# Meowuu7/equi-articulated-pose

Measured on AMD Instinct MI355X. Metric: point-clouds/sec (4096 pts, 60 anchors) fwd+bwd, higher is better.
Workload: dtype f32; 1 GPU; 8 x 4096-pt synthetic laptop clouds per GPU, 3-block inter backbone 1->64->128->512 (NN=64,K=24,A=60), forward+backward+Adam; clouds_per_gpu=8, points=4096, anchors=60

## Files before the change

### equi-articulated-pose_amd/vgtk/_hip.py

```python
import ctypes
import os
import weakref

import torch

_PKG_ROOT = os.path.abspath(os.path.join(os.path.dirname(__file__), '..'))
LIB_PATH = os.path.join(_PKG_ROOT, 'libeap_hip.so')

if not os.path.exists(LIB_PATH):
    raise ImportError(
        f'{LIB_PATH} not found: build the HIP extension first '
        '(python -c "import __graft_entry__ as g; g.build()" or make -C equi-articulated-pose_amd/csrc). '
        'This package has no CPU fallback.')

lib = ctypes.CDLL(LIB_PATH)
lib.eap_last_error.restype = ctypes.c_char_p
lib.eap_last_kernel.restype = ctypes.c_char_p
lib.eap_gemm_f32_reduce_workspace.restype = ctypes.c_int64
lib.eap_so3_inter_group_bwd_workspace.restype = ctypes.c_int64
lib.eap_inter_zpconv_fwd_workspace.restype = ctypes.c_int64
lib.eap_inter_zpconv_bwd_workspace.restype = ctypes.c_int64
lib.eap_inter_zpconv_bwd_hot_workspace.restype = ctypes.c_int64
lib.eap_bn_act_segments.restype = ctypes.c_int

# ... 761 lines not shown
        return hint[0].sum(1, dtype=torch.float64), hint[1].sum(1, dtype=torch.float64)
    ps, pq = _partials(x, b, c, n)
    call('eap_bn_stats_f32', x, b, c, _I64(n), _ptr(x), _ptr(ps), _ptr(pq))
    return ps.sum(1, dtype=torch.float64), pq.sum(1, dtype=torch.float64)


def bn_act_fwd(x, b, c, n, scale, shift, slope, residual=None):
    y = torch.empty_like(x)
    if residual is None:
        call('eap_bn_act_fwd_f32', x, b, c, _I64(n), _F32(slope), _ptr(x), _ptr(scale), _ptr(shift), _ptr(y))
    else:
        call('eap_bn_act_add_fwd_f32', x, b, c, _I64(n), _F32(slope), _ptr(x), _ptr(scale), _ptr(shift), _ptr(residual), _ptr(y))
    return y


def bn_act_bwd_reduce(gy, x, b, c, n, scale, shift, mean, invstd, slope):
    pg, pgx = _partials(x, b, c, n)
    call('eap_bn_act_bwd_reduce_f32', x, b, c, _I64(n), _F32(slope), _ptr(gy), _ptr(x), _ptr(scale), _ptr(shift),
         _ptr(mean), _ptr(invstd), _ptr(pg), _ptr(pgx))
    return pg.sum(1, dtype=torch.float64), pgx.sum(1, dtype=torch.float64)


_ROWMAX_HINT = [None]
USE_ROWMAX_HINT = True
ROWMAX_HINTS_TAKEN = 0


def leave_rowmax_hint(t, rowmax):
    _leave_hint(_ROWMAX_HINT, t, rowmax)


def take_rowmax_hint(t):
    global ROWMAX_HINTS_TAKEN
    rowmax = _take_hint(_ROWMAX_HINT, t)
    ROWMAX_HINTS_TAKEN += rowmax is not None
    return rowmax


def bn_act_bwd_apply(gy, x, b, c, n, scale, shift, mean, invstd, k2, k3, slope):
    gx = torch.empty_like(x)
    if x.dim() == 4 and x.shape[3] % 4 == 0 and x.shape[3] <= 64 and n == x.shape[2] * x.shape[3] and c % 128 == 0 and gx.data_ptr() % 16 == 0 \
            and gy.data_ptr() % 16 == 0 and x.data_ptr() % 16 == 0:
        rowmax = torch.empty(b, c, x.shape[3], dtype=torch.int32, device=x.device)
        call('eap_bn_act_bwd_apply_rowmax_f32', x, b, c, _I64(n), int(x.shape[3]), _F32(slope), _ptr(gy), _ptr(x), _ptr(scale), _ptr(shift),
             _ptr(mean), _ptr(invstd), _ptr(k2), _ptr(k3), _ptr(gx), _ptr(rowmax))
        leave_rowmax_hint(gx, rowmax)
        return gx
    call('eap_bn_act_bwd_apply_f32', x, b, c, _I64(n), _F32(slope), _ptr(gy), _ptr(x), _ptr(scale), _ptr(shift),
         _ptr(mean), _ptr(invstd), _ptr(k2), _ptr(k3), _ptr(gx))
    return gx



def bn_stats_masked(x, b, c, n, na, mask):
    ps, pq = _partials(x, b, c, n)
    call('eap_bn_stats_masked_f32', x, b, c, _I64(n), na, _ptr(x), _ptr(mask), _ptr(ps), _ptr(pq))
    return ps.view(c, b, -1).sum(2, dtype=torch.float64).t(), pq.view(c, b, -1).sum(2, dtype=torch.float64).t()


def bn_act_cloud_fwd(x, b, c, n, scale, shift, slope):
    y = torch.empty_like(x)
    call('eap_bn_act_cloud_fwd_f32', x, b, c, _I64(n), _F32(slope), _ptr(x), _ptr(scale), _ptr(shift), _ptr(y))
    return y


def bn_act_cloud_bwd_reduce(gy, x, b, c, n, scale, shift, mean, invstd, slope):
    pg, pgx = _partials(x, b, c, n)
    call('eap_bn_act_cloud_bwd_reduce_f32', x, b, c, _I64(n), _F32(slope), _ptr(gy), _ptr(x), _ptr(scale), _ptr(shift),
         _ptr(mean), _ptr(invstd), _ptr(pg), _ptr(pgx))
    return pg.view(c, b, -1).sum(2, dtype=torch.float64).t(), pgx.view(c, b, -1).sum(2, dtype=torch.float64).t()


def bn_act_cloud_bwd_apply(gy, x, b, c, n, na, scale, shift, mean, invstd, k2, k3, mask, slope):
    gx = torch.empty_like(x)
    call('eap_bn_act_cloud_bwd_apply_f32', x, b, c, _I64(n), na, _F32(slope), _ptr(gy), _ptr(x), _ptr(scale), _ptr(shift),
         _ptr(mean), _ptr(invstd), _ptr(k2), _ptr(k3), _ptr(mask), _ptr(gx))
    return gx


def so3_intra_conv(feats, W, intra_idx32):
    b, c, p, na = feats.shape
    o, nt = W.shape[0], intra_idx32.shape[1]
    out = torch.empty(b, o, p, na, dtype=torch.float32, device=feats.device)
    split = SPLIT_BF16_CONTRACTION and W.data_ptr() % 16 == 0 and lib.eap_so3_intra_conv_bf16x3_f32_supported(b, o, c, p, na, nt)
    tag = {'flops': 2.0 * b * o * c * nt * p * na, 'shape': ('intra_conv', b, o, c, p, na, nt)}
    if split and SPLIT_PLANES == 2 and feats.data_ptr() % 16 == 0:
        abs_w = absmax_rows(W, 1, o, c * nt, c * nt, 0)
        abs_f = absmax_colgroups(feats, b, c, p * na, p * na, c * p * na, na) if na % 4 == 0 else None
        if abs_w is not None and abs_f is not None:
            call('eap_so3_intra_conv_f16x2_f32', out, b, o, c, p, na, nt, _ptr(W), _ptr(feats), _ptr(intra_idx32), _ptr(out), _ptr(abs_w),
                 _ptr(abs_f), tag=tag)
            return out
    call('eap_so3_intra_conv_bf16x3_f32' if split else 'eap_so3_intra_conv_f32', out, b, o, c, p, na, nt, _ptr(W), _ptr(feats),
         _ptr(intra_idx32), _ptr(out), tag=tag)
    return out
```

### equi-articulated-pose_amd/vgtk/so3conv/functional.py

```python
import math
import os
import weakref

import numpy as np
import torch

import vgtk
import vgtk.functional as fr
import vgtk.pc as pctk
import vgtk.spconv as zpconv
import vgtk.cuda.grouping as cuda_nn

from .. import _hip

inter_so3conv_feat_grouping = zpconv.inter_zpconv_grouping_naive
batched_index_select = zpconv.batched_index_select
batched_index_select_other = zpconv.batched_index_select_other

MATERIALIZE_INTER_W = False

GAMMA_SIZE = 3
ROOT = vgtk.__path__[0]
Rs, R_idx, canonical_relative = fr.icosahedron_so3(GAMMA_SIZE)
_KP = np.load(os.path.join(ROOT, 'data', 'anchors', 'constants.npz'))
# ... 412 lines not shown

def _inverse_lists(idx, gx, n_sup, ident, nonident=None):
    if nonident is None:
        nonident = (gx[..., 3].contiguous().view(torch.int32) != ident).flatten(1).any(1).to(torch.int32)
    head = _ListHead(idx, n_sup, nonident)
    rcap, any_nonident = head.decide()
    head.wait()
    ent_p, ent_gx = _hip.inv_lists_fill(idx, gx, head.rows, head.off, rcap)
    return (head.rows[:, :rcap].contiguous(), head.off[:, :rcap].contiguous(), head.cnt[:, :rcap].contiguous(),
            ent_p, ent_gx, rcap, not any_nonident)


X_LAYOUT = 'transposed'


X_CHUNK_CLOUDS = 8
_KEEP_X_HINT = {}


def _keep_x_hint(W):
    hit = _KEEP_X_HINT.get(id(W))
    return bool(hit is not None and hit[0]() is W and hit[1])


def _set_keep_x_hint(W, keep):
    if len(_KEEP_X_HINT) > 1024:
        _KEEP_X_HINT.clear()
    _KEEP_X_HINT[id(W)] = (weakref.ref(W), bool(keep))


class FoldedEpilogue:

    def __init__(self, scale, shift, slope, residual=None):
        self.scale, self.shift, self.slope, self.residual = scale.contiguous(), shift.contiguous(), float(slope), residual
        self.applied = False
        self.inference = not torch.is_grad_enabled()


class TrainEpilogue:

    def __init__(self, norm):
        self.norm = norm
        self.applied = False
        self.inference = False
        self.residual = None

    def moments(self, s1, s2, pivot, count):
        from .blocks import affine_from_moments, batch_moments, update_running_stats
        norm = self.norm
        mean, var, total = batch_moments(s1, s2, pivot, count, norm.sync)
        if norm.running_mean is not None:
            update_running_stats(norm.running_mean, norm.running_var, mean, var, total, norm.momentum)
        gamma = norm.weight.detach().double()
        scale, shift, _ = affine_from_moments(mean, var, gamma, norm.bias.detach(), norm.eps)
        inv_gamma = torch.where(gamma == 0, torch.zeros_like(gamma), 1.0 / gamma).float()
        self.saved = (scale, norm.bias.detach().float().clone(), inv_gamma.contiguous(), total)
        return scale.contiguous(), shift.contiguous(), float(norm.negative_slope)


def _contract_into(W, x, y, layout, epilogue=None, b0=0, x_bound=None):
    b, c, ks, p, na = x.shape
    o = W.shape[0]
    if layout == 2:
        xt = x.view(b, p * na, c * ks).transpose(1, 2)
    if epilogue is not None and layout == 2:
        res = None if epilogue.residual is None else epilogue.residual[b0:b0 + b]
        if _hip.matmul_epilogue(W, xt, y, epilogue.scale, epilogue.shift, epilogue.slope, res, b_bound=x_bound):
            epilogue.applied = True
            return
        if b0 > 0 and epilogue.applied:
            raise RuntimeError('folded epilogue: the slabs of one contraction took different kernels')
    if layout == 2:
        _hip.matmul(W, xt, y, b_bound=x_bound)
    elif layout == 1:
        _hip.gemm(0, 0, o, p * na, c * ks, W, c * ks, 0, x, p * na, c * ks * p * na, y, p * na, o * p * na, b, b_blocked=True)
    else:
        _hip.matmul(W, x.view(b, c * ks, p * na), y)


def _grouped_bound(feats, idx):
    if not (_hip.SPLIT_BF16_CONTRACTION and _hip.SPLIT_PLANES == 2):
        return None
    return _hip.so3_grouped_bound(feats, idx)


BACKWARD_LOG = None
FORWARD_LOG = None


DENSE_MODE = os.environ.get('EAP_DENSE', 'auto')
DENSE_ROW_FACTOR = 5.0
DENSE_MAX_GROUPS = 16.0
DENSE_MAX_GROUPS_WIDE = 16.0
DENSE_FWD_NARROW = True
FUSE_CONV_NORM = True


def _dense_rows(rcap, n):
    return (rcap + 15) & ~15


def _dense_wanted(head, o, p, na, ks, nn, n):
    if DENSE_MODE == 'off' or head is None or head.memb is None:
        return 0, False
    rcap, _ = head.decide()
    rp = _dense_rows(rcap, n)
    if rp <= 0 or rp > n or not head.dense_possible() or not _hip.so3_dense_supported(p, na, ks, rp, o):
# ... 212 lines not shown
    moments = affine = None
    if train_ep is not None:
        ep, moments = train_ep, train_ep.moments
    elif folded is not None and folded.residual is None:
        ep, affine = folded, (folded.scale, folded.shift, folded.slope)
    else:
        return _dense_forward(feats, W, rows, geo, p), None
    g, ldg, operand = _dense_operand(feats, W, rows, geo)
    y = _hip.so3_dense_fwd_bnact(g, geo, p, feats.shape[1], ldg, moments, operand=operand, o=W.shape[0], affine=affine)
    ep.applied = True
    return y, (None if train_ep is None else train_ep.saved + (float(train_ep.norm.negative_slope), bool(train_ep.norm.sync)))


def _forward_lists(feats, W, args, layout, keep, folded, head, fill):
    idx, gx, rk, mult, sigma, nonident = args.idx, args.gx, args.rk, args.mult, args.sigma, args.nonident
    b, c, n, na = feats.shape
    p, ks, o = idx.shape[1], rk.shape[1], W.shape[0]
    if fill:
        head.fill(idx, gx, n)
    y = torch.empty(b, o, p, na, dtype=torch.float32, device=feats.device)
    coset = _coset_tables(mult, args.ident) if (mult is not None and nonident is not None and layout == 2) else None
    x_bound = _grouped_bound(feats, idx) if layout == 2 else None
    step = max(1, b if keep else X_CHUNK_CLOUDS)
    tp = (not keep and STORE_ORDER_COLUMNS and layout == 2 and _hip.so3_group_fwd_tp_takes(c, na, ks)
          and (mult is None or (coset is not None and _hip.so3_group_perm_lists2_takes(c, na, ks, n))))
    Wc = W.index_select(1, _hip.so3_group_fwd_tp_columns(c, ks, W.device)) if tp else W
    x = None
    for b0 in range(0, b, step):
        b1 = min(b, b0 + step)
        x = _hip.so3_inter_group_fwd(feats[b0:b1], idx[b0:b1], gx[b0:b1], rk, mult, sigma,
                                     None if nonident is None else nonident[b0:b1], blocked=layout, coset=coset, store_order=tp)
        _contract_into(Wc, x, y[b0:b1].view(b1 - b0, o, p * na), layout, folded, b0,
                       x_bound=None if x_bound is None else (x_bound[b0:b1], na, 1.0))
        x = x if keep else None
    return y, x


def _forward_map(feats, W, args, keep, folded):
    idx, gx, rk, amap = args.idx, args.gx, args.rk, args.amap
    b, na = feats.shape[0], feats.shape[3]
    p, o = idx.shape[1], W.shape[0]
    y = torch.empty(b, o, p, na, dtype=torch.float32, device=feats.device)
    step = max(1, b if keep else X_CHUNK_CLOUDS)
    x = None
    for b0 in range(0, b, step):
        b1 = min(b, b0 + step)
        x = _hip.so3_inter_group_fwd_map(feats[b0:b1], idx[b0:b1], gx[b0:b1], rk, amap[b0:b1], args.sigma)
        _contract_into(W, x, y[b0:b1].view(b1 - b0, o, p * na), 0, folded, b0)
        x = x if keep else None
    return y, x



def _weight_operand(W, c, ks, pad_c=None):
    o = W.shape[0]
    W2 = W.view(o, c, ks).permute(1, 0, 2).reshape(c, o * ks).contiguous()
    if pad_c is not None and pad_c != c:
        W2 = torch.cat([W2, torch.zeros(pad_c - c, o * ks, dtype=torch.float32, device=W.device)])
    return W2


def _rows_grad_from_z(z, W2, c, rp, na, ldz, anchor_major, z_bound=None, reorder=None):
    b, (pad_c, oks) = z.shape[0], W2.shape
    gFc = torch.empty(b, pad_c, ldz, dtype=torch.float32, device=z.device)
    _hip.matmul(W2, z.view(b, oks, ldz), gFc, b_bound=z_bound)
    if anchor_major:
        return gFc[:, :c, :rp * na].reshape(b, c, na, rp).transpose(2, 3)
    gFc = gFc.view(b, c, rp, na)
    return gFc if reorder is None else _hip.anchor_reorder(gFc, reorder)


def _weight_grad_rows(z, fc4, o, ks, ldz, anchor_major, reorder=None):
    b, c, rp, na = fc4.shape
    if reorder is not None:
        fc4 = _hip.anchor_reorder(fc4, reorder)
    fc = fc4.transpose(2, 3).contiguous() if anchor_major else fc4
    return _weight_grad_from_z(z, fc.view(b, c, rp * na), b, c, o, ks, rp * na, ldz)



def _backward_dense(gy, W, feats, head, geo, bn, yact, need_f, need_w):
    b, c, n, na = feats.shape
    o, ks, p, rp = W.shape[0], geo.ks, gy.shape[2], geo.rp
    if BACKWARD_LOG is not None:
        BACKWARD_LOG.append({'channels': (c, o), 'support_rows': n, 'referenced_rows_max': int(rp), 'regime': 'dense rows',
                             **({'norm': 'in the node'} if bn is not None else {})})
    ra = na * rp
    pad_c = 128 if (c == 64 and bn is not None) else c
    ldz = _hip.dense_pitch(ra) if (pad_c % 128 == 0 and (o * ks) % 16 == 0 and need_f) else ra
    gF = gW = g_bn_w = g_bn_b = z_bound = None
    if bn is not None:
        k1, beta, inv_gamma, count, slope, sync = bn
        from .blocks import all_reduce_sums
        sg, sgx, gmax, xmax = _hip.bn_act_bwd_reduce_fromy(gy, yact, beta, inv_gamma, slope)
        g_bn_w, g_bn_b = sgx.float(), sg.float()
        tg, tgx = all_reduce_sums(sg, sgx, sync=sync)
        k2 = (k1.double() * tg / count).float()
        k3 = (k1.double() * tgx / count).float()
        coef = torch.stack([k1, k2, k3, beta, inv_gamma]).contiguous()
        bound = (k1.abs()[None, :, None] * gmax + k2.abs()[None, :, None] + k3.abs()[None, :, None] * xmax).contiguous()
        z = _hip.so3_dense_bwd_bn(gy, yact, geo, ldz, coef, bound, slope)
        if ldz % 4 == 0 and rp % 4 == 0:
            live = torch.arange(rp, device=gy.device)[None, :] < head.n_rows[:, None]
            cntf = torch.where(live, head.cnt[:, :rp], torch.zeros_like(head.cnt[:, :rp])).clamp(min=0, max=p).to(torch.float32)
            cols = bound.amax(1)[:, :, None] * cntf[:, None, :]
            words = torch.zeros(b, ldz // 4, dtype=torch.float32, device=gy.device)
# ... 88 lines not shown
        gx_ = torch.empty_like(x.view(b, ck, pa))
        Wt = W.t().contiguous()
        _hip.matmul(Wt, gy.view(b, o, pa), gx_)
        gF = _hip.so3_inter_group_bwd(gx_.view(b, c, ks, p, na), idx, gx, rk, mult, args.sigma, n, args.ident)
    return gF, gW


def _backward_map(gy, W, feats, x, args, need_f, need_w):
    b, c, n, na = feats.shape
    idx, gx, rk, amap = args.idx, args.gx, args.rk, args.amap
    p, ks = idx.shape[1], rk.shape[1]
    o, ck, pa = W.shape[0], c * ks, p * na
    gF = gW = None
    if need_w:
        if x is None:
            x = _hip.so3_inter_group_fwd_map(feats, idx, gx, rk, amap, args.sigma)
        gW = torch.empty_like(W)
        _hip.matmul_reduce(gy.view(b, o, pa), x.view(b, ck, pa).transpose(1, 2), gW)
    if need_f:
        gx_ = torch.empty(b, ck, pa, dtype=torch.float32, device=gy.device)
        Wt = W.t().contiguous()
        _hip.matmul(Wt, gy.view(b, o, pa), gx_)
        gF = _hip.so3_inter_group_bwd_map(gx_.view(b, c, ks, p, na), idx, gx, rk, amap, args.sigma, n)
    return gF, gW


class _InterConv(torch.autograd.Function):

    DIFFERENTIABLE = 4

    @staticmethod
    def forward(ctx, feats, W_param, bn_weight, bn_bias, args):
        feats = feats.contiguous()
        W = W_param.contiguous()
        idx, rk, mult, nonident = args.idx, args.rk, args.mult, args.nonident
        can = X_LAYOUT != 'reference' and _hip.so3_inter_group_fwd_can_block(
            feats.shape[1], feats.shape[2], feats.shape[3], rk.shape[1], mult is not None, nonident is not None)
        layout = 0 if not can else (2 if X_LAYOUT == 'transposed' else 1)
        _, c, n, na = feats.shape
        p, ks, o = idx.shape[1], rk.shape[1], W.shape[0]
        needs_grad = (ctx.needs_input_grad[0] or ctx.needs_input_grad[1]) and args.grad_mode
        train_ep = args.epilogue if isinstance(args.epilogue, TrainEpilogue) else None
        folded = None if train_ep is not None else args.epilogue
        if folded is not None and (needs_grad or not folded.inference):
            raise RuntimeError('a folded epilogue is an inference-time fusion: build and use it under torch.no_grad()')
        if args.amap is not None:
            if FORWARD_LOG is not None:
                FORWARD_LOG.append({'channels': (c, o), 'dense': False, 'parts': None, 'regime': 'anchor map'})
            y, x = _forward_map(feats, W, args, needs_grad and ctx.needs_input_grad[1], folded)
            ctx.bn, ctx.conv_args, ctx.head, ctx.layout, ctx.plan = None, args, None, 0, None
            ctx.W_param = weakref.ref(W_param)
            ctx.save_for_backward(W, x, idx, args.gx, rk, None, nonident, feats, None)
            return y
        lists_ok = BACKWARD_MODE != 'dx' and _inv_lists_supported(idx, n, na, ks)
        keep = needs_grad and (not lists_ok or _keep_x_hint(W_param))
        plan = _DensePlan(args, n, o, lists_ok, needs_grad, keep, folded)
        head = plan.head if needs_grad else None
        if FORWARD_LOG is not None:
            FORWARD_LOG.append({'channels': (c, o), 'dense': bool(plan.forward), 'parts': None if plan.parts is None else plan.parts.n})
        if plan.forward:
            bn_only = args.grad_mode and not needs_grad and (ctx.needs_input_grad[2] or ctx.needs_input_grad[3])
            y, ctx.bn = _forward_dense(feats, W, plan, p, train_ep if (FUSE_CONV_NORM and not bn_only) else None, folded)
            x, layout = None, 0
        else:
            fill = head is not None and plan.probed and not keep and plan.rp == 0
            y, x = _forward_lists(feats, W, args, layout, keep, folded, head, fill)
            ctx.bn = None
        ctx.conv_args, ctx.head, ctx.layout = args, head, layout
        ctx.plan = plan if (plan.rp > 0 and needs_grad) else None
        ctx.W_param = weakref.ref(W_param)
        ctx.save_for_backward(W, x, idx, args.gx, rk, mult, nonident, feats, y if (ctx.bn is not None and needs_grad) else None)
        return y

    @staticmethod
    def backward(ctx, gy):
        W, x, idx, gx, rk, mult, nonident, feats, yact = ctx.saved_tensors
        args, head, plan = ctx.conv_args, ctx.head, ctx.plan
        gy = gy.contiguous()
        n = feats.shape[2]
        need_f, need_w = ctx.needs_input_grad[0], ctx.needs_input_grad[1]
        g_bn_w = g_bn_b = None
        if args.amap is not None:
            if BACKWARD_LOG is not None:
                BACKWARD_LOG.append({'channels': (feats.shape[1], W.shape[0]), 'support_rows': n, 'referenced_rows_max': 0, 'regime': 'anchor map'})
            gF, gW = _backward_map(gy, W, feats, x, args, need_f, need_w)
        elif plan is not None and plan.parts is not None:
            gF, gW = _backward_dense_parts(gy, W, feats, head, plan.geo(), need_f, need_w)
        elif plan is not None:
            gF, gW, g_bn_w, g_bn_b = _backward_dense(gy, W, feats, head, plan.geo(), ctx.bn, yact, need_f, need_w)
        else:
            rcap, any_nonident = 0, True
            if head is not None:
                rcap, any_nonident = head.decide()
                if BACKWARD_MODE == 'auto' and rcap * INV_ROW_FRACTION > n:
                    head.entries = None
                    head = None
            if BACKWARD_LOG is not None:
                BACKWARD_LOG.append({'channels': (feats.shape[1], W.shape[0]), 'support_rows': n, 'referenced_rows_max': int(rcap),
                                     'regime': 'inverse lists' if head is not None else 'textbook dX'})
            Wp = ctx.W_param()
            if Wp is not None:
                _set_keep_x_hint(Wp, head is None)
            if head is not None:
                gF, gW = _backward_lists(gy, W, feats, idx, gx, rk, mult, args, head, rcap, any_nonident, need_f, need_w)
            else:
                gF, gW = _backward_textbook(gy, W, feats, x, idx, gx, rk, mult, nonident, args, ctx.layout, need_f, need_w)
        return (gF, gW, g_bn_w, g_bn_b) + (None,) * (len(ctx.needs_input_grad) - _InterConv.DIFFERENTIABLE)


INTRA_DW_SLICE = 64


class _IntraConv(torch.autograd.Function):

    @staticmethod
    def forward(ctx, feats, W, idx32):
        feats, W = feats.contiguous(), W.contiguous()
        ctx.save_for_backward(feats, W, idx32)
        return _hip.so3_intra_conv(feats, W, idx32)

    @staticmethod
    def backward(ctx, gy):
        feats, W, idx32 = ctx.saved_tensors
        gy = gy.contiguous()
        b, c, p, na = feats.shape
        o, nt = W.shape[0], idx32.shape[1]
        gF = gW = None
        if ctx.needs_input_grad[0]:
            inv = torch.empty_like(idx32)
            inv.scatter_(0, idx32.long(), torch.arange(na, device=idx32.device, dtype=torch.int32)[:, None].expand(na, nt).contiguous())
            W2 = W.view(o, c, nt).permute(1, 0, 2).reshape(c, o * nt).contiguous()
            gF = _hip.so3_intra_conv(gy, W2, inv.contiguous())
        if ctx.needs_input_grad[1]:
            gW = torch.empty(o, c, nt, dtype=torch.float32, device=gy.device)
            pa = p * na
# ... 319 lines not shown
```

### include/eap_hip.h

```cpp
#ifndef EAP_HIP_H
#define EAP_HIP_H

#include <stdint.h>

#ifdef __cplusplus
extern "C" {
#endif

typedef void *eap_stream_t;

const char *eap_last_error(void);
int eap_launch_dims_ok(int64_t gx, int64_t gy, int64_t gz, int bx, int by, int bz);
const char *eap_last_kernel(void);
int eap_abi_version(void);


int eap_ball_query_f32(int b, int n, int m, float radius, int nsample, const float *new_xyz,
                       const float *xyz, int32_t *idx, eap_stream_t stream);
int eap_ball_query_f64(int b, int n, int m, float radius, int nsample, const double *new_xyz,
                       const double *xyz, int32_t *idx, eap_stream_t stream);

int eap_furthest_point_sampling_f32(int b, int n, int m, const float *xyz, float *temp,
                                    int32_t *idx, eap_stream_t stream);
int eap_furthest_point_sampling_f64(int b, int n, int m, const double *xyz, double *temp,
// ... 277 lines not shown


int eap_chamfer_fwd_f32(int b, int n, int m, const float *xyz1, const float *xyz2, float *dist1,
                        float *dist2, int32_t *idx1, int32_t *idx2, eap_stream_t stream);
int eap_chamfer_fwd_f64(int b, int n, int m, const double *xyz1, const double *xyz2, double *dist1,
                        double *dist2, int32_t *idx1, int32_t *idx2, eap_stream_t stream);
int eap_chamfer_bwd_f32(int b, int n, int m, const float *xyz1, const float *xyz2,
                        const int32_t *idx1, const int32_t *idx2, const float *g1, const float *g2,
                        float *gxyz1, float *gxyz2, eap_stream_t stream);
int eap_chamfer_bwd_ordered_f32(int b, int n, int m, const float *xyz1, const float *xyz2,
                                const int32_t *idx1, const int32_t *idx2, const float *g1, const float *g2,
                                float *gxyz1, float *gxyz2, eap_stream_t stream);
int eap_chamfer_bwd_ordered_f64(int b, int n, int m, const double *xyz1, const double *xyz2,
                                const int32_t *idx1, const int32_t *idx2, const double *g1, const double *g2,
                                double *gxyz1, double *gxyz2, eap_stream_t stream);

int eap_bn_act_segments(int64_t n);
int eap_bn_stats_f32(int b, int c, int64_t n, const float *x, float *psum, float *psq, eap_stream_t stream);
int eap_bn_act_fwd_f32(int b, int c, int64_t n, float slope, const float *x, const float *scale,
                       const float *shift, float *y, eap_stream_t stream);
int eap_bn_act_add_fwd_f32(int b, int c, int64_t n, float slope, const float *x, const float *scale,
                           const float *shift, const float *res, float *y, eap_stream_t stream);
int eap_bn_act_bwd_reduce_f32(int b, int c, int64_t n, float slope, const float *gy, const float *x,
                              const float *scale, const float *shift, const float *mean,
                              const float *invstd, float *pg, float *pgx, eap_stream_t stream);
int eap_bn_act_bwd_apply_f32(int b, int c, int64_t n, float slope, const float *gy, const float *x,
                             const float *scale, const float *shift, const float *mean,
                             const float *invstd, const float *k2, const float *k3, float *gx,
                             eap_stream_t stream);
int eap_bn_act_bwd_apply_rowmax_f32(int b, int c, int64_t n, int na, float slope, const float *gy, const float *x,
                                    const float *scale, const float *shift, const float *mean, const float *invstd,
                                    const float *k2, const float *k3, float *gx, uint32_t *rowmax, eap_stream_t stream);
int eap_bn_act_fromy_blocks(int64_t n, int na);
int eap_bn_act_bwd_reduce_fromy_f32(int b, int c, int64_t n, int na, float slope, const float *gy, const float *y, const float *beta,
                                    const float *inv_gamma, float *pg, float *pgx, uint32_t *gmax, uint32_t *xmax, eap_stream_t stream);

int eap_bn_stats_masked_f32(int b, int c, int64_t n, int na, const float *x, const float *mask, float *psum, float *psq,
                            eap_stream_t stream);
int eap_bn_act_cloud_fwd_f32(int b, int c, int64_t n, float slope, const float *x, const float *scale, const float *shift,
                             float *y, eap_stream_t stream);
int eap_bn_act_cloud_bwd_reduce_f32(int b, int c, int64_t n, float slope, const float *gy, const float *x, const float *scale,
                                    const float *shift, const float *mean, const float *invstd, float *pg, float *pgx,
                                    eap_stream_t stream);
int eap_bn_act_cloud_bwd_apply_f32(int b, int c, int64_t n, int na, float slope, const float *gy, const float *x,
                                   const float *scale, const float *shift, const float *mean, const float *invstd,
                                   const float *k2, const float *k3, const float *mask, float *gx, eap_stream_t stream);

int eap_narrow_contract_supported(int b, int o, int c, int64_t n);
int eap_narrow_contract_fwd_f32(int b, int o, int c, int64_t n, const float *W, const float *x, float *y, eap_stream_t stream);
int eap_narrow_contract_dx_f32(int b, int o, int c, int64_t n, const float *W, const float *g, float *dx, eap_stream_t stream);
int eap_narrow_contract_dw_slabs(int64_t n);
int eap_narrow_contract_dw_f32(int b, int o, int c, int64_t n, const float *g, const float *x, float *partial, eap_stream_t stream);

int eap_anchor_attn_pool_fwd_f32(int b, int c, int n, int na, float temperature, const float *x, const float *logits,
                                 float *out, float *conf, eap_stream_t stream);
int eap_anchor_attn_pool_bwd_f32(int b, int c, int n, int na, float temperature, const float *x, const float *logits,
                                 const float *g, float *dx, float *dlogits, eap_stream_t stream);
int eap_slot_masked_mean_fwd_f32(int b, int ns, int c, int n, int na, const float *x, const float *mask,
                                 const float *inv_den, float *out, eap_stream_t stream);
int eap_slot_masked_mean_bwd_f32(int b, int ns, int c, int n, int na, const float *g, const float *mask,
                                 const float *inv_den, float *dx, eap_stream_t stream);
int eap_masked_max_fwd_f32(int b, int c, int n, int na, const float *x, const float *mask, float *out, int32_t *arg,
                           eap_stream_t stream);
int eap_masked_max_bwd_f32(int b, int c, int n, int na, const float *g, const int32_t *arg, const float *mask, float *dx,
                           eap_stream_t stream);

#ifdef __cplusplus
}
#endif
#endif
```

Measured before the change: 163.3 point-clouds/sec.

## Fuse narrow-input inter conv with batch norm and activation, recomputing conv output

Adds a path for the first inter conv block, where the input has few channels (C*K at most 32) and no input gradient is needed. The contraction is done with MFMA tiles, and batch-norm statistics, the normalize plus leaky-ReLU epilogue, the backward reductions and the weight gradient are fused around it. The conv output is recomputed in each kernel instead of being stored and read back, which cuts the memory traffic of the wide pre-norm activation at the cost of redoing the cheap contraction. It adds several new kernels and a per-segment partial reduction for the weight gradient.

```diff
diff --git a/equi-articulated-pose_amd/csrc/narrow_conv.hip b/equi-articulated-pose_amd/csrc/narrow_conv.hip
--- /dev/null
+++ b/equi-articulated-pose_amd/csrc/narrow_conv.hip
@@ -0,0 +1,370 @@
+#include "common.h"
+#include "device_prims.h"
+#include <type_traits>
+
+namespace {
+
+constexpr int NT = 256, WAVES = 4;
+constexpr int TILE = 128;
+constexpr int SEGC = 2048;
+
+__device__ __forceinline__ int drow(int r, int h) { return (r & 3) + 8 * (r >> 2) + 4 * h; }
+
+template <int KS2>
+__device__ __forceinline__ void load_x(f32x4 (&xa)[KS2], const float *__restrict__ xb, long n, long col0, unsigned voff, bool ok, int ck, int h) {
+#pragma unroll
+    for (int s = 0; s < KS2; ++s)
+        xa[s] = (ok && 2 * s + h < ck) ? ld_off<f32x4>(xb + (size_t)(2 * s) * n + col0, voff) : (f32x4){0.f, 0.f, 0.f, 0.f};
+}
+
+template <int KS2>
+__device__ __forceinline__ void load_w(float (&wf)[KS2], const float *__restrict__ W, int orow, int ck, int h) {
+#pragma unroll
+    for (int s = 0; s < KS2; ++s) wf[s] = (2 * s + h < ck) ? W[(size_t)orow * ck + 2 * s + h] : 0.f;
+}
+
+template <int KS2, bool T>
+__device__ __forceinline__ void conv_tile(f32x16 (&d)[4], const f32x4 (&xa)[KS2], const float (&wf)[KS2]) {
+#pragma unroll
+    for (int c = 0; c < 4; ++c)
+#pragma unroll
+        for (int r = 0; r < 16; ++r) d[c][r] = 0.f;
+#pragma unroll
+    for (int s = 0; s < KS2; ++s) {
+        if (T) {
+            d[0] = __builtin_amdgcn_mfma_f32_32x32x2f32(xa[s].x, wf[s], d[0], 0, 0, 0);
+            d[1] = __builtin_amdgcn_mfma_f32_32x32x2f32(xa[s].y, wf[s], d[1], 0, 0, 0);
+            d[2] = __builtin_amdgcn_mfma_f32_32x32x2f32(xa[s].z, wf[s], d[2], 0, 0, 0);
+            d[3] = __builtin_amdgcn_mfma_f32_32x32x2f32(xa[s].w, wf[s], d[3], 0, 0, 0);
+        } else {
+            d[0] = __builtin_amdgcn_mfma_f32_32x32x2f32(wf[s], xa[s].x, d[0], 0, 0, 0);
+            d[1] = __builtin_amdgcn_mfma_f32_32x32x2f32(wf[s], xa[s].y, d[1], 0, 0, 0);
+            d[2] = __builtin_amdgcn_mfma_f32_32x32x2f32(wf[s], xa[s].z, d[2], 0, 0, 0);
+            d[3] = __builtin_amdgcn_mfma_f32_32x32x2f32(wf[s], xa[s].w, d[3], 0, 0, 0);
+        }
+    }
+}
+
+__device__ __forceinline__ void block_sums(float (&sa)[16], float (&qa)[16], float (*s_red)[2][32], int ct, int o0, int bi, int nb,
+                                           int nseg, int seg, float *__restrict__ pa, float *__restrict__ pq) {
+    const int t = threadIdx.x, lane = t & 63, wave = t >> 6, li = lane & 31, h = lane >> 5;
+#pragma unroll
+    for (int r = 0; r < 16; ++r) {
+        float a = sa[r], q = qa[r];
+#pragma unroll
+        for (int d = 16; d > 0; d >>= 1) { a += __shfl_xor(a, d); q += __shfl_xor(q, d); }
+        if (li == 0) { s_red[wave][0][drow(r, h)] = a; s_red[wave][1][drow(r, h)] = q; }
+    }
+    __syncthreads();
+    if (t < 32 * ct) {
+        float a = 0.f, q = 0.f;
+        for (int w = t >> 5; w < WAVES; w += ct) { a += s_red[w][0][t & 31]; q += s_red[w][1][t & 31]; }
+        const size_t at = ((size_t)(o0 + t) * nb + bi) * nseg + seg;
+        pa[at] = a; pq[at] = q;
+    }
+}
+
+struct Pos {
+    int seg, bi, lane, li, h, ch0, cw, ncw;
+    long beg, end;
+    unsigned xoff;
+    __device__ Pos(int ct, long n) {
+        seg = blockIdx.x; bi = blockIdx.z;
+        const int wave = threadIdx.x >> 6;
+        lane = threadIdx.x & 63; li = lane & 31; h = lane >> 5;
+        ch0 = (blockIdx.y * ct + wave % ct) * 32; cw = wave / ct; ncw = WAVES / ct;
+        beg = (long)seg * SEGC; end = min(n, beg + SEGC);
+        xoff = 4u * ((unsigned)h * (unsigned)n + 4u * li);
+    }
+};
+
+template <int KS2>
+__global__ __launch_bounds__(NT) void narrow_conv_stats_kernel(int ct, int ck, long n, int nseg, const float *__restrict__ W,
+                                                                 const float *__restrict__ x, float *__restrict__ pivot,
+                                                                 float *__restrict__ psum, float *__restrict__ psq) {
+    __shared__ __attribute__((aligned(16))) float s_piv[64];
+    __shared__ float s_red[WAVES][2][32];
+    const Pos w(ct, n);
+    const int t = threadIdx.x, o0 = blockIdx.y * ct * 32, h = w.h;
+    if (t < 32 * ct) {
+        float p = 0.f;
+        for (int k = 0; k < ck; ++k) p = fmaf(W[(size_t)(o0 + t) * ck + k], x[(size_t)k * n], p);
+        s_piv[t] = p;
+        if (w.seg == 0 && w.bi == 0) pivot[o0 + t] = p;
+    }
+    __syncthreads();
+    float wf[KS2];
+    load_w<KS2>(wf, W, w.ch0 + w.li, ck, h);
+    f32x4 pv[4];
+#pragma unroll
+    for (int g = 0; g < 4; ++g) pv[g] = *reinterpret_cast<const f32x4 *>(&s_piv[w.ch0 - o0 + 8 * g + 4 * h]);
+    float sa[16], qa[16];
+#pragma unroll
+    for (int r = 0; r < 16; ++r) sa[r] = qa[r] = 0.f;
+    const float *xb = x + (size_t)w.bi * ck * n;
+#pragma unroll 1
+    for (long col0 = w.beg + (long)w.cw * TILE; col0 < w.end; col0 += (long)w.ncw * TILE) {
+        const long col = col0 + 4 * w.li;
+        const bool ok = col < n;
+        f32x4 xa[KS2];
+        load_x<KS2>(xa, xb, n, col0, w.xoff, ok, ck, h);
+        f32x16 d[4];
+        conv_tile<KS2, false>(d, xa, wf);
+        if (ok) {
+#pragma unroll
+            for (int r = 0; r < 16; ++r)
+#pragma unroll
+                for (int c = 0; c < 4; ++c) {
+                    const float dd = d[c][r] - pv[r >> 2][r & 3];
+                    sa[r] += dd;
+                    qa[r] = fmaf(dd, dd, qa[r]);
+                }
+        }
+    }
+    block_sums(sa, qa, s_red, ct, o0, w.bi, gridDim.z, nseg, w.seg, psum, psq);
+}
+
+template <int KS2>
+__global__ __launch_bounds__(NT) void narrow_conv_bnact_fwd_kernel(int ct, int o, int ck, long n, float slope, const float *__restrict__ W,
+                                                                     const float *__restrict__ x, const float *__restrict__ scale,
+                                                                     const float *__restrict__ shift, float *__restrict__ y) {
+    const Pos w(ct, n);
+    const int h = w.h;
+    float wf[KS2];
+    load_w<KS2>(wf, W, w.ch0 + w.li, ck, h);
+    f32x4 sc[4], sh[4];
+#pragma unroll
+    for (int g = 0; g < 4; ++g) {
+        sc[g] = *reinterpret_cast<const f32x4 *>(scale + w.ch0 + 8 * g + 4 * h);
+        sh[g] = *reinterpret_cast<const f32x4 *>(shift + w.ch0 + 8 * g + 4 * h);
+    }
+    const float *xb = x + (size_t)w.bi * ck * n;
+    float *yb = y + ((size_t)w.bi * o + w.ch0) * n;
+    const unsigned roff = 4u * (4u * h * (unsigned)n + 4u * w.li);
+#pragma unroll 1
+    for (long col0 = w.beg + (long)w.cw * TILE; col0 < w.end; col0 += (long)w.ncw * TILE) {
+        const long col = col0 + 4 * w.li;
+        const bool ok = col < n;
+        f32x4 xa[KS2];
+        load_x<KS2>(xa, xb, n, col0, w.xoff, ok, ck, h);
+        f32x16 d[4];
+        conv_tile<KS2, false>(d, xa, wf);
+        if (ok) {
+#pragma unroll
+            for (int r = 0; r < 16; ++r) {
+                const float a = sc[r >> 2][r & 3], b = sh[r >> 2][r & 3];
+                f32x4 v;
+                v.x = fmaf(d[0][r], a, b); v.y = fmaf(d[1][r], a, b); v.z = fmaf(d[2][r], a, b); v.w = fmaf(d[3][r], a, b);
+                v.x = v.x > 0.f ? v.x : v.x * slope; v.y = v.y > 0.f ? v.y : v.y * slope;
+                v.z = v.z > 0.f ? v.z : v.z * slope; v.w = v.w > 0.f ? v.w : v.w * slope;
+                st_off<f32x4>(yb + (size_t)(8 * (r >> 2)) * n + col0, roff + 4u * (unsigned)(r & 3) * (unsigned)n, v);
+            }
+        }
+    }
+}
+
+template <int KS2>
+__global__ __launch_bounds__(NT) void narrow_conv_bwd_reduce_kernel(int ct, int o, int ck, long n, int nseg, float slope,
+                                                                      const float *__restrict__ gy, const float *__restrict__ x,
+                                                                      const float *__restrict__ W, const float *__restrict__ scale,
+                                                                      const float *__restrict__ shift, const float *__restrict__ mean,
+                                                                      const float *__restrict__ invstd, float *__restrict__ pg,
+                                                                      float *__restrict__ pgx) {
+    __shared__ __attribute__((aligned(16))) float s_sc[64], s_sh[64], s_mu[64], s_is[64];
+    __shared__ float s_red[WAVES][2][32];
+    const Pos w(ct, n);
+    const int t = threadIdx.x, o0 = blockIdx.y * ct * 32, h = w.h;
+    if (t < 32 * ct) { s_sc[t] = scale[o0 + t]; s_sh[t] = shift[o0 + t]; s_mu[t] = mean[o0 + t]; s_is[t] = invstd[o0 + t]; }
+    __syncthreads();
+    float wf[KS2];
+    load_w<KS2>(wf, W, w.ch0 + w.li, ck, h);
+    float sa[16], qa[16];
+#pragma unroll
+    for (int r = 0; r < 16; ++r) sa[r] = qa[r] = 0.f;
+    const float *xb = x + (size_t)w.bi * ck * n;
+    const float *gb = gy + ((size_t)w.bi * o + w.ch0) * n;
+    const unsigned roff = 4u * (4u * h * (unsigned)n + 4u * w.li);
+    const int lc = w.ch0 - o0;
+#pragma unroll 1
+    for (long col0 = w.beg + (long)w.cw * TILE; col0 < w.end; col0 += (long)w.ncw * TILE) {
+        const long col = col0 + 4 * w.li;
+        const bool ok = col < n;
+        f32x4 xa[KS2];
+        load_x<KS2>(xa, xb, n, col0, w.xoff, ok, ck, h);
+        f32x16 d[4];
+        conv_tile<KS2, false>(d, xa, wf);
+        if (ok) {
+#pragma unroll
+            for (int g = 0; g < 4; ++g) {
+                f32x4 gv[4];
+#pragma unroll
+                for (int q = 0; q < 4; ++q) gv[q] = ld_off<f32x4>(gb + (size_t)(8 * g) * n + col0, roff + 4u * q * (unsigned)n);
+                const f32x4 sc = *reinterpret_cast<const f32x4 *>(&s_sc[lc + 8 * g + 4 * h]), sh = *reinterpret_cast<const f32x4 *>(&s_sh[lc + 8 * g + 4 * h]);
+                const f32x4 mu = *reinterpret_cast<const f32x4 *>(&s_mu[lc + 8 * g + 4 * h]), is = *reinterpret_cast<const f32x4 *>(&s_is[lc + 8 * g + 4 * h]);
+#pragma unroll
+                for (int q = 0; q < 4; ++q)
+#pragma unroll
+                    for (int c = 0; c < 4; ++c) {
+                        const float yv = d[c][4 * g + q];
+                        const float pre = fmaf(yv, sc[q], sh[q]);
+                        const float gg = pre > 0.f ? gv[q][c] : gv[q][c] * slope;
+                        sa[4 * g + q] += gg;
+                        qa[4 * g + q] = fmaf(gg, (yv - mu[q]) * is[q], qa[4 * g + q]);
+                    }
+            }
+        }
+    }
+    block_sums(sa, qa, s_red, ct, o0, w.bi, gridDim.z, nseg, w.seg, pg, pgx);
+}
+
+template <int KS2>
+__global__ __launch_bounds__(NT) void narrow_conv_bwd_dw_kernel(int ct, int o, int ck, long n, int nseg, float slope,
+                                                                  const float *__restrict__ gy, const float *__restrict__ x,
+                                                                  const float *__restrict__ W, const float *__restrict__ scale,
+                                                                  const float *__restrict__ shift, const float *__restrict__ mean,
+                                                                  const float *__restrict__ invstd, const float *__restrict__ k2,
+                                                                  const float *__restrict__ k3, float *__restrict__ partial) {
+    __shared__ float s_part[WAVES][16][64];
+    const Pos w(ct, n);
+    const int h = w.h, li = w.li, wave = threadIdx.x >> 6;
+    const int ch = w.ch0 + li;
+    float wf[KS2];
+    load_w<KS2>(wf, W, ch, ck, h);
+    const float sc = scale[ch], sh = shift[ch], mu = mean[ch], is = invstd[ch], c2 = k2[ch], c3 = k3[ch];
+    const float *gb = gy + ((size_t)w.bi * o + w.ch0) * n;
+    const unsigned goff = 4u * ((unsigned)li * (unsigned)n + 16u * h), koff = 4u * ((unsigned)min(li, ck - 1) * (unsigned)n + 16u * h);
+    f32x16 dw;
+#pragma unroll
+    for (int r = 0; r < 16; ++r) dw[r] = 0.f;
+    const float *xb = x + (size_t)w.bi * ck * n;
+    const f32x4 zero4 = {0.f, 0.f, 0.f, 0.f};
+#pragma unroll 1
+    for (long col0 = w.beg + (long)w.cw * TILE; col0 < w.end; col0 += (long)w.ncw * TILE) {
+        const long col = col0 + 4 * li;
+        f32x4 xa[KS2];
+        load_x<KS2>(xa, xb, n, col0, w.xoff, col < n, ck, h);
+        f32x16 d[4];
+        conv_tile<KS2, true>(d, xa, wf);
+#pragma unroll
+        for (int g = 0; g < 4; ++g) {
+            f32x4 gv[4], xv[4];
+#pragma unroll
+            for (int q = 0; q < 4; ++q) {
+                const long cq = col0 + 4 * (8 * g + 4 * h + q);
+                const bool in = cq < n;
+                gv[q] = in ? ld_off<f32x4>(gb + col0 + 4 * (8 * g + q), goff) : zero4;
+                xv[q] = (in && li < ck) ? ld_off<f32x4>(xb + col0 + 4 * (8 * g + q), koff) : zero4;
+            }
+#pragma unroll
+            for (int q = 0; q < 4; ++q)
+#pragma unroll
+                for (int c = 0; c < 4; ++c) {
+                    const float yv = d[c][4 * g + q];
+                    const float pre = fmaf(yv, sc, sh);
+                    const float gg = pre > 0.f ? gv[q][c] : gv[q][c] * slope;
+                    const float gx = fmaf(gg, sc, -c2) - ((yv - mu) * is) * c3;
+                    dw = __builtin_amdgcn_mfma_f32_32x32x2f32(gx, xv[q][c], dw, 0, 0, 0);
+                }
+        }
+    }
+#pragma unroll
+    for (int r = 0; r < 16; ++r) s_part[wave][r][w.lane] = dw[r];
+    __syncthreads();
+    if (wave < ct) {
+        float *slab = partial + ((size_t)w.bi * nseg + w.seg) * o * ck;
+#pragma unroll
+        for (int r = 0; r < 16; ++r) {
+            float v = 0.f;
+            for (int u = wave; u < WAVES; u += ct) v += s_part[u][r][w.lane];
+            if (li < ck) slab[(size_t)(w.ch0 + drow(r, h)) * ck + li] = v;
+        }
+    }
+}
+
+__global__ __launch_bounds__(256) void narrow_conv_dw_sum_kernel(int mn, int slabs, const float *__restrict__ partial, float *__restrict__ dW) {
+    const int e = blockIdx.x * 4 + (threadIdx.x >> 6), lane = threadIdx.x & 63;
+    if (e >= mn) return;
+    float s = 0.f;
+    for (int z = lane; z < slabs; z += 64) s += partial[(size_t)z * mn + e];
+#pragma unroll
+    for (int d = 32; d > 0; d >>= 1) s += __shfl_xor(s, d);
+    if (lane == 0) dW[e] = s;
+}
+
+inline int nseg_of(long n) { return (int)((n + SEGC - 1) / SEGC); }
+
+inline bool misaligned(const void *p) { return (reinterpret_cast<uintptr_t>(p) & 15) != 0; }
+
+inline int refuse(const char *who, int o, int ck, long n, const void *p0, const void *p1, const void *p2 = nullptr) {
+    char buf[200];
+    const char *why = nullptr;
+    if (ck < 1 || ck > 32) why = "1 to 32 contraction indices (C*K)";
+    else if (o < 32 || o % 32 != 0) why = "a multiple of 32 output channels";
+    else if (n < 0 || (n & 3) != 0 || n >= (1l << 25)) why = "a row length (P*A) that is a multiple of 4 below 2^25";
+    else if (misaligned(p0) || misaligned(p1) || misaligned(p2)) why = "16-byte aligned tensors";
+    if (!why) return 0;
+    snprintf(buf, sizeof(buf), "%s: takes %s", who, why);
+    return eap::bad_arg(buf);
+}
+
+inline int tiles_per_block(int o) { return o % 64 == 0 ? 2 : 1; }
+
+template <typename F>
+int by_depth(int ck, F &&f) {
+    return ck <= 24 ? f(std::integral_constant<int, 12>{}) : f(std::integral_constant<int, 16>{});
+}
+
+}
+
+extern "C" int eap_narrow_conv_segments(int64_t n) { return n > 0 ? nseg_of((long)n) : 0; }
+
+extern "C" int eap_narrow_conv_stats_f32(int b, int o, int ck, int64_t n, const float *W, const float *x, float *pivot, float *psum,
+                                         float *psq, eap_stream_t stream) {
+    if (int e = refuse("narrow_conv_stats", o, ck, (long)n, x, nullptr)) return e;
+    if (b <= 0 || n <= 0) return 0;
+    const int nseg = nseg_of((long)n), ct = tiles_per_block(o);
+    return by_depth(ck, [&](auto ks2) {
+        return eap::run_kernel("narrow_conv_stats", narrow_conv_stats_kernel<decltype(ks2)::value>, nseg, o / (32 * ct), b, dim3(NT), 0, eap::S(stream), ct,
+                               ck, (long)n, nseg, W, x, pivot, psum, psq);
+    });
+}
+
+extern "C" int eap_narrow_conv_bnact_fwd_f32(int b, int o, int ck, int64_t n, float slope, const float *W, const float *x, const float *scale,
+                                             const float *shift, float *y, eap_stream_t stream) {
+    if (int e = refuse("narrow_conv_bnact_fwd", o, ck, (long)n, x, y, scale)) return e;
+    if (misaligned(shift)) return eap::bad_arg("narrow_conv_bnact_fwd: takes 16-byte aligned tensors");
+    if (b <= 0 || n <= 0) return 0;
+    const int ct = tiles_per_block(o);
+    return by_depth(ck, [&](auto ks2) {
+        return eap::run_kernel("narrow_conv_bnact_fwd", narrow_conv_bnact_fwd_kernel<decltype(ks2)::value>, nseg_of((long)n), o / (32 * ct), b, dim3(NT), 0,
+                               eap::S(stream), ct, o, ck, (long)n, slope, W, x, scale, shift, y);
+    });
+}
+
+extern "C" int eap_narrow_conv_bwd_reduce_f32(int b, int o, int ck, int64_t n, float slope, const float *gy, const float *x, const float *W,
+                                              const float *scale, const float *shift, const float *mean, const float *invstd, float *pg,
+                                              float *pgx, eap_stream_t stream) {
+    if (int e = refuse("narrow_conv_bwd_reduce", o, ck, (long)n, x, gy)) return e;
+    if (b <= 0 || n <= 0) return 0;
+    const int nseg = nseg_of((long)n), ct = tiles_per_block(o);
+    return by_depth(ck, [&](auto ks2) {
+        return eap::run_kernel("narrow_conv_bwd_reduce", narrow_conv_bwd_reduce_kernel<decltype(ks2)::value>, nseg, o / (32 * ct), b, dim3(NT), 0, eap::S(stream),
+                               ct, o, ck, (long)n, nseg, slope, gy, x, W, scale, shift, mean, invstd, pg, pgx);
+    });
+}
+
+extern "C" int eap_narrow_conv_bwd_dw_f32(int b, int o, int ck, int64_t n, float slope, const float *gy, const float *x, const float *W,
+                                          const float *scale, const float *shift, const float *mean, const float *invstd, const float *k2,
+                                          const float *k3, float *partial, float *dW, eap_stream_t stream) {
+    if (int e = refuse("narrow_conv_bwd_dw", o, ck, (long)n, x, gy)) return e;
+    if (b <= 0 || n <= 0) return 0;
+    const int nseg = nseg_of((long)n), ct = tiles_per_block(o);
+    hipStream_t s = eap::S(stream);
+    int e = by_depth(ck, [&](auto ks2) {
+        return eap::run_kernel("narrow_conv_bwd_dw", narrow_conv_bwd_dw_kernel<decltype(ks2)::value>, nseg, o / (32 * ct), b, dim3(NT), 0, s, ct, o, ck, (long)n,
+                               nseg, slope, gy, x, W, scale, shift, mean, invstd, k2, k3, partial);
+    });
+    if (e) return e;
+    const int mn = o * ck;
+    return eap::run_kernel("narrow_conv_bwd_dw (sum)", narrow_conv_dw_sum_kernel, eap::cdiv(mn, 4), 1, 1, dim3(256), 0, s, mn, b * nseg, partial, dW);
+}
diff --git a/equi-articulated-pose_amd/vgtk/_hip.py b/equi-articulated-pose_amd/vgtk/_hip.py
--- a/equi-articulated-pose_amd/vgtk/_hip.py
+++ b/equi-articulated-pose_amd/vgtk/_hip.py
@@ -837,6 +837,61 @@
 
 
 
+NARROW_CONV_MAX_CK = 32
+
+
+def narrow_conv_takes(o, ck, n):
+    return 1 <= ck <= NARROW_CONV_MAX_CK and o >= 32 and o % 32 == 0 and n % 4 == 0 and n < (1 << 25)
+
+
+def _narrow_partials(x, b, o, n):
+    nseg = int(lib.eap_narrow_conv_segments(_I64(n)))
+    return (torch.empty(o, b * nseg, dtype=torch.float32, device=x.device),
+            torch.empty(o, b * nseg, dtype=torch.float32, device=x.device))
+
+
+def narrow_conv_stats(W, x):
+    check_input(W, x)
+    b, ck, n = x.shape
+    o = W.shape[0]
+    ps, pq = _narrow_partials(x, b, o, n)
+    pivot = torch.empty(o, dtype=torch.float32, device=x.device)
+    call('eap_narrow_conv_stats_f32', x, b, o, ck, _I64(n), _ptr(W), _ptr(x), _ptr(pivot), _ptr(ps), _ptr(pq))
+    return ps.sum(1, dtype=torch.float64), pq.sum(1, dtype=torch.float64), pivot.double()
+
+
+def narrow_conv_bnact_fwd(W, x, scale, shift, slope):
+    check_input(W, x, scale, shift)
+    b, ck, n = x.shape
+    o = W.shape[0]
+    y = torch.empty(b, o, n, dtype=torch.float32, device=x.device)
+    call('eap_narrow_conv_bnact_fwd_f32', x, b, o, ck, _I64(n), _F32(slope), _ptr(W), _ptr(x), _ptr(scale), _ptr(shift), _ptr(y))
+    return y
+
+
+def narrow_conv_bwd_reduce(gy, x, W, scale, shift, mean, invstd, slope):
+    check_input(gy, x, W, scale, shift, mean, invstd)
+    b, ck, n = x.shape
+    o = W.shape[0]
+    pg, pgx = _narrow_partials(x, b, o, n)
+    call('eap_narrow_conv_bwd_reduce_f32', x, b, o, ck, _I64(n), _F32(slope), _ptr(gy), _ptr(x), _ptr(W), _ptr(scale), _ptr(shift),
+         _ptr(mean), _ptr(invstd), _ptr(pg), _ptr(pgx))
+    return pg.sum(1, dtype=torch.float64), pgx.sum(1, dtype=torch.float64)
+
+
+def narrow_conv_bwd_dw(gy, x, W, scale, shift, mean, invstd, k2, k3, slope):
+    check_input(gy, x, W, scale, shift, mean, invstd, k2, k3)
+    b, ck, n = x.shape
+    o = W.shape[0]
+    nseg = int(lib.eap_narrow_conv_segments(_I64(n)))
+    partial = torch.empty(b * nseg, o, ck, dtype=torch.float32, device=x.device)
+    dW = torch.empty(o, ck, dtype=torch.float32, device=x.device)
+    call('eap_narrow_conv_bwd_dw_f32', x, b, o, ck, _I64(n), _F32(slope), _ptr(gy), _ptr(x), _ptr(W), _ptr(scale), _ptr(shift),
+         _ptr(mean), _ptr(invstd), _ptr(k2), _ptr(k3), _ptr(partial), _ptr(dW))
+    return dW
+
+
+
 def bn_stats_masked(x, b, c, n, na, mask):
     ps, pq = _partials(x, b, c, n)
     call('eap_bn_stats_masked_f32', x, b, c, _I64(n), na, _ptr(x), _ptr(mask), _ptr(ps), _ptr(pq))
diff --git a/equi-articulated-pose_amd/vgtk/so3conv/functional.py b/equi-articulated-pose_amd/vgtk/so3conv/functional.py
--- a/equi-articulated-pose_amd/vgtk/so3conv/functional.py
+++ b/equi-articulated-pose_amd/vgtk/so3conv/functional.py
@@ -488,7 +488,8 @@
         if norm.running_mean is not None:
             update_running_stats(norm.running_mean, norm.running_var, mean, var, total, norm.momentum)
         gamma = norm.weight.detach().double()
-        scale, shift, _ = affine_from_moments(mean, var, gamma, norm.bias.detach(), norm.eps)
+        scale, shift, invstd = affine_from_moments(mean, var, gamma, norm.bias.detach(), norm.eps)
+        self.stats = (mean, invstd)
         inv_gamma = torch.where(gamma == 0, torch.zeros_like(gamma), 1.0 / gamma).float()
         self.saved = (scale, norm.bias.detach().float().clone(), inv_gamma.contiguous(), total)
         return scale.contiguous(), shift.contiguous(), float(norm.negative_slope)
@@ -807,6 +808,35 @@
 
 
 
+def _forward_narrow(feats, W, args, train_ep):
+    idx, rk = args.idx, args.rk
+    b, c, _, na = feats.shape
+    p, ks, o = idx.shape[1], rk.shape[1], W.shape[0]
+    x = _hip.so3_inter_group_fwd(feats, idx, args.gx, rk, args.mult, args.sigma, args.nonident).view(b, c * ks, p * na)
+    s1, s2, pivot = _hip.narrow_conv_stats(W, x)
+    scale, shift, slope = train_ep.moments(s1, s2, pivot, b * p * na)
+    y = _hip.narrow_conv_bnact_fwd(W, x, scale, shift, slope).view(b, o, p, na)
+    train_ep.applied = True
+    mean, invstd = train_ep.stats
+    return y, x, (scale, shift, mean.float(), invstd.float(), train_ep.saved[3], slope, bool(train_ep.norm.sync))
+
+
+def _backward_narrow(gy, W, x, bn, need_w):
+    from .blocks import all_reduce_sums
+    scale, shift, mean, invstd, count, slope, sync = bn
+    b, o = gy.shape[0], gy.shape[1]
+    gy = gy.view(b, o, -1)
+    sg, sgx = _hip.narrow_conv_bwd_reduce(gy, x, W, scale, shift, mean, invstd, slope)
+    gW = None
+    if need_w:
+        tg, tgx = all_reduce_sums(sg, sgx, sync=sync)
+        k2 = (scale.double() * tg / count).float()
+        k3 = (scale.double() * tgx / count).float()
+        gW = _hip.narrow_conv_bwd_dw(gy, x, W, scale, shift, mean, invstd, k2, k3, slope)
+    return gW, sgx.float(), sg.float()
+
+
+
 def _weight_operand(W, c, ks, pad_c=None):
     o = W.shape[0]
     W2 = W.view(o, c, ks).permute(1, 0, 2).reshape(c, o * ks).contiguous()
@@ -1001,7 +1031,18 @@
             ctx.W_param = weakref.ref(W_param)
             ctx.save_for_backward(W, x, idx, args.gx, rk, None, nonident, feats, None)
             return y
-        lists_ok = BACKWARD_MODE != 'dx' and _inv_lists_supported(idx, n, na, ks)
+        narrow = c * ks <= _hip.NARROW_CONV_MAX_CK and not ctx.needs_input_grad[0]
+        if narrow and train_ep is not None and FUSE_CONV_NORM and _hip.narrow_conv_takes(o, c * ks, p * na):
+            if FORWARD_LOG is not None:
+                FORWARD_LOG.append({'channels': (c, o), 'dense': False, 'parts': None, 'regime': 'narrow input'})
+            y, x, bn = _forward_narrow(feats, W, args, train_ep)
+            wanted = args.grad_mode and any(ctx.needs_input_grad[1:_InterConv.DIFFERENTIABLE])
+            ctx.bn, ctx.conv_args, ctx.head, ctx.layout, ctx.plan = (bn if wanted else None), args, None, 0, None
+            ctx.narrow = True
+            ctx.W_param = weakref.ref(W_param)
+            ctx.save_for_backward(W, x if wanted else None, idx, None, rk, None, None, feats, None)
+            return y
+        lists_ok = BACKWARD_MODE != 'dx' and _inv_lists_supported(idx, n, na, ks) and not narrow
         keep = needs_grad and (not lists_ok or _keep_x_hint(W_param))
         plan = _DensePlan(args, n, o, lists_ok, needs_grad, keep, folded)
         head = plan.head if needs_grad else None
@@ -1029,7 +1070,13 @@
         n = feats.shape[2]
         need_f, need_w = ctx.needs_input_grad[0], ctx.needs_input_grad[1]
         g_bn_w = g_bn_b = None
-        if args.amap is not None:
+        if getattr(ctx, 'narrow', False):
+            if BACKWARD_LOG is not None:
+                BACKWARD_LOG.append({'channels': (feats.shape[1], W.shape[0]), 'support_rows': n, 'referenced_rows_max': 0,
+                                     'regime': 'narrow input', 'norm': 'in the node'})
+            gF = None
+            gW, g_bn_w, g_bn_b = _backward_narrow(gy, W, x, ctx.bn, need_w)
+        elif args.amap is not None:
             if BACKWARD_LOG is not None:
                 BACKWARD_LOG.append({'channels': (feats.shape[1], W.shape[0]), 'support_rows': n, 'referenced_rows_max': 0, 'regime': 'anchor map'})
             gF, gW = _backward_map(gy, W, feats, x, args, need_f, need_w)
diff --git a/include/eap_hip.h b/include/eap_hip.h
--- a/include/eap_hip.h
+++ b/include/eap_hip.h
@@ -353,6 +353,18 @@
 int eap_narrow_contract_dw_slabs(int64_t n);
 int eap_narrow_contract_dw_f32(int b, int o, int c, int64_t n, const float *g, const float *x, float *partial, eap_stream_t stream);
 
+int eap_narrow_conv_segments(int64_t n);
+int eap_narrow_conv_stats_f32(int b, int o, int ck, int64_t n, const float *W, const float *x, float *pivot, float *psum, float *psq,
+                              eap_stream_t stream);
+int eap_narrow_conv_bnact_fwd_f32(int b, int o, int ck, int64_t n, float slope, const float *W, const float *x, const float *scale,
+                                  const float *shift, float *y, eap_stream_t stream);
+int eap_narrow_conv_bwd_reduce_f32(int b, int o, int ck, int64_t n, float slope, const float *gy, const float *x, const float *W,
+                                   const float *scale, const float *shift, const float *mean, const float *invstd, float *pg, float *pgx,
+                                   eap_stream_t stream);
+int eap_narrow_conv_bwd_dw_f32(int b, int o, int ck, int64_t n, float slope, const float *gy, const float *x, const float *W,
+                               const float *scale, const float *shift, const float *mean, const float *invstd, const float *k2,
+                               const float *k3, float *partial, float *dW, eap_stream_t stream);
+
 int eap_anchor_attn_pool_fwd_f32(int b, int c, int n, int na, float temperature, const float *x, const float *logits,
                                  float *out, float *conf, eap_stream_t stream);
 int eap_anchor_attn_pool_bwd_f32(int b, int c, int n, int na, float temperature, const float *x, const float *logits,
```

After: 165.7 point-clouds/sec, median of 6. +1.5%, better.
